# Sanoojan/VFace

Hardware: AMD Instinct MI355X
Metric: swapped frames/sec at 512x512, 50-step DDIM (higher is better)
Workload: dtype f16

## Files before the change

### include/vface_hip.h

```cpp
#ifndef VFACE_HIP_H
#define VFACE_HIP_H

#include <stddef.h>
#include <stdint.h>

#ifdef __cplusplus
extern "C" {
#endif

#define VFACE_ABI_VERSION 8

#define VFACE_OK 0
#define VFACE_ERR_ARG (-1)
#define VFACE_ERR_ALIGN (-2)
#define VFACE_ERR_SHAPE (-3)
#define VFACE_ERR_DTYPE (-4)
#define VFACE_ERR_LAUNCH (-5)
#define VFACE_ERR_WORKSPACE (-6)

#define VFACE_F16 0
#define VFACE_BF16 1

#define VFACE_EPI_GEGLU 1
#define VFACE_EPI_OUT_F32 2
// ... 65 lines not shown

int vface_layernorm(const void* x, int64_t ldx, const float* gamma, const float* beta, void* y, int64_t ldy, int M,
                    int C, float eps, int in_f32, int dtype, void* stream);

int vface_groupnorm_partial_floats(int nimg, int hw, int C, int groups);
int vface_groupnorm_stats(const void* x, int64_t ldx, int nimg, int hw, int C, int groups, float eps, float* partial,
                          float* stats, int in_f32, int dtype, void* stream);
int vface_groupnorm_finalize_cols(const float* colstats, int64_t ld_colstats, int nimg, int hw, int C, int groups, float eps,
                                  float* stats, void* stream);
int vface_groupnorm_coeffs_from_cols(const float* colstats, int64_t ld_colstats, int nimg, int hw, int C, int groups, float eps,
                                     const float* gamma, const float* beta, float* ab, void* stream);
int vface_groupnorm_apply(const void* x, int64_t ldx, const float* stats, const float* gamma, const float* beta,
                          void* y, int64_t ldy, int nimg, int hw, int C, int groups, int silu, int in_f32, int dtype,
                          void* stream);

int vface_flow_warp(const void* src, int64_t ld_src, int64_t fs_src, const void* prev, int64_t ld_prev,
                    const float* flow, const float* flow_prev, void* dst, int64_t ld_dst, int64_t fs_dst, int F,
                    int h, int w, int C, float alpha, float one_minus_alpha, int flags, int32_t* dbg_x0,
                    int32_t* dbg_y0, int dtype, void* stream);

int vface_flow_to_latent(const float* flow_px, float* out, int pairs, int H, int W, int factor, void* stream);

int vface_im2col(const void* X, int64_t ldx, int nimg, int H, int W, int C, int KH, int KW, int stride, int pad_y, int pad_x, void* out,
                 int64_t ldo, int dtype, void* stream);

int64_t vface_channel_stats_partial_floats(int nimg, int hw, int C);
int vface_channel_stats(const void* x, int64_t ldx, int nimg, int hw, int C, float eps, float* partial, float* stats, int dtype,
                        void* stream);

int vface_channel_norm_act(const void* x, int64_t ldx, const float* stats, const void* residual, int64_t ldr, void* y, int64_t ldy,
// ... 125 lines not shown
```

### vface_amd/csrc/capi.cpp

```cpp
#include "../../include/vface_hip.h"

#include <hip/hip_runtime.h>

#include "vface_kernels.hpp"

namespace {
inline hipStream_t S(void* s) { return reinterpret_cast<hipStream_t>(s); }

GemmParams plain_gemm(const void* A, long lda, const void* Wt, long ldw, int M, int N, int K, const float* bias,
                      void* C, long ldc, const void* zeros) {
    GemmParams p{};
    p.mode = 0; p.A = A; p.lda = lda; p.Wt = Wt; p.ldw = ldw; p.Kw = K; p.M = M; p.N = N; p.K = K;
    p.bias = bias; p.C = C; p.ldc = ldc; p.zeros = zeros;
    return p;
}
inline void apply_s32(GemmParams& p, const vface_stream32* s) {
    if (!s) return;
    if (s->residual32) { p.residual = s->residual32; p.ldr = s->ldr32; p.res_f32 = 1; }
    if (s->out32) { p.C32 = s->out32; p.ldc32 = s->ldo32; }
    if (s->in_scale_shift) { p.gn_ab = s->in_scale_shift; p.ld_gn_ab = s->ld_scale_shift; p.gn_silu = s->in_silu ? 1 : 0; }
}
}

extern "C" {
// ... 138 lines not shown
                                  float* stats, void* stream) {
    return vf_launch_gn_finalize_cols(colstats, ld_colstats, nimg, hw, C, groups, eps, stats, S(stream));
}

int vface_groupnorm_coeffs_from_cols(const float* colstats, int64_t ld_colstats, int nimg, int hw, int C, int groups, float eps,
                                     const float* gamma, const float* beta, float* ab, void* stream) {
    return vf_launch_gn_coeffs_cols(colstats, ld_colstats, nimg, hw, C, groups, eps, gamma, beta, ab, S(stream));
}

int vface_groupnorm_apply(const void* x, int64_t ldx, const float* stats, const float* gamma, const float* beta,
                          void* y, int64_t ldy, int nimg, int hw, int C, int groups, int silu, int in_f32, int dtype,
                          void* stream) {
    return vf_launch_gn_apply(x, ldx, stats, gamma, beta, y, ldy, nimg, hw, C, groups, silu, in_f32, dtype, S(stream));
}

int vface_flow_warp(const void* src, int64_t ld_src, int64_t fs_src, const void* prev, int64_t ld_prev,
                    const float* flow, const float* flow_prev, void* dst, int64_t ld_dst, int64_t fs_dst, int F,
                    int h, int w, int C, float alpha, float one_minus_alpha, int flags, int32_t* dbg_x0,
                    int32_t* dbg_y0, int dtype, void* stream) {
    return vf_launch_flow_warp(src, ld_src, fs_src, prev, ld_prev, flow, flow_prev, dst, ld_dst, fs_dst, F, h, w, C,
                               alpha, one_minus_alpha, flags, dbg_x0, dbg_y0, dtype, S(stream));
}

int vface_flow_to_latent(const float* flow_px, float* out, int pairs, int H, int W, int factor, void* stream) {
    return vf_launch_flow_to_latent(flow_px, out, pairs, H, W, factor, S(stream));
}

int vface_im2col(const void* X, int64_t ldx, int nimg, int H, int W, int C, int KH, int KW, int stride, int pad_y, int pad_x, void* out,
                 int64_t ldo, int dtype, void* stream) {
    return vf_launch_im2col(X, ldx, nimg, H, W, C, KH, KW, stride, pad_y, pad_x, out, ldo, dtype, S(stream));
// ... 256 lines not shown
```

### vface_amd/csrc/outconv.hip

```cpp
#include <type_traits>

#include "common.hpp"
#include "vface_kernels.hpp"

namespace {

constexpr int OC_TX = 16, OC_TY = 8;
constexpr int OC_PX = OC_TX + 2, OC_PY = OC_TY + 2;
constexpr int OC_THREADS = 512;
constexpr int OC_ITEMS = OC_PX * OC_PY * 8;
constexpr int OC_NIT = (OC_ITEMS + OC_THREADS - 1) / OC_THREADS;
constexpr int OC_MAXC = 640;
constexpr int OC_PITCH = 64 + 8;

template <class TT, bool IN32, int COUT>
__global__ __launch_bounds__(OC_THREADS) void gn_silu_conv3x3_small_kernel(OutConvParams p) {
    using E = typename TT::elem;
    using V8 = typename TT::v8;
    __shared__ __attribute__((aligned(16))) E patch[OC_PX * OC_PY * OC_PITCH];
    __shared__ float sAB[2 * OC_MAXC];
    static_assert(sizeof(patch) >= 3 * OC_TX * OC_TY * 4 * sizeof(float), "the partial sums are reduced through the patch");
    const int t = threadIdx.x;
    const int tiles_x = (p.W + OC_TX - 1) / OC_TX, tiles_y = (p.H + OC_TY - 1) / OC_TY;
    const int img = blockIdx.x / (tiles_x * tiles_y), tl = blockIdx.x - img * (tiles_x * tiles_y);
    const int ty0 = (tl / tiles_x) * OC_TY, tx0 = (tl % tiles_x) * OC_TX;
    const int pix = t & 127, py = pix >> 4, px = pix & 15;
    const int slice = __builtin_amdgcn_readfirstlane(t >> 7);
    const int oy = ty0 + py, ox = tx0 + px;
    const long img_row0 = (long)img * p.H * p.W;
    float acc[COUT];
#pragma unroll
    for (int o = 0; o < COUT; ++o) acc[o] = 0.f;
    const unsigned* wq = reinterpret_cast<const unsigned*>(p.Wt);
    const int nchunks = p.Cin / 64;
    for (int ch = t; ch < p.Cin; ch += OC_THREADS) {
        const float2 ab = *reinterpret_cast<const float2*>(p.ab + ((long)img * p.ld_ab + ch) * 2);
        sAB[ch] = ab.x; sAB[OC_MAXC + ch] = ab.y;
    }
    using RAW = typename std::conditional<IN32, float4, V8>::type;
    RAW raw[OC_NIT][IN32 ? 2 : 1];
    auto item_row = [&](int i, long& row) -> bool {
        const int it = t + i * OC_THREADS, pp = it >> 3;
        const int iy = ty0 - 1 + pp / OC_PX, ix = tx0 - 1 + pp % OC_PX;
        row = img_row0 + (long)iy * p.W + ix;
        return it < OC_ITEMS && iy >= 0 && iy < p.H && ix >= 0 && ix < p.W;
    };
    auto load_chunk = [&](int c) {
#pragma unroll
// ... 26 lines not shown
                    v[0] = a.x; v[1] = a.y; v[2] = a.z; v[3] = a.w; v[4] = b.x; v[5] = b.y; v[6] = b.z; v[7] = b.w;
                } else {
#pragma unroll
                    for (int j = 0; j < 8; ++j) v[j] = to_f32(raw[i][0][j]);
                }
#pragma unroll
                for (int j = 0; j < 8; ++j) {
                    const float f = v[j] * sAB[c * 64 + g8 * 8 + j] + sAB[OC_MAXC + c * 64 + g8 * 8 + j];
                    o[j] = from_f32<E>(silu_f(f));
                }
            }
            *reinterpret_cast<V8*>(patch + pp * OC_PITCH + g8 * 8) = o;
        }
    };
    load_chunk(0);
    __syncthreads();
    for (int c = 0; c < nchunks; ++c) {
        store_chunk(c);
        __syncthreads();
        if (c + 1 < nchunks) load_chunk(c + 1);
#pragma unroll
        for (int tap = 0; tap < 9; ++tap) {
            const E* pr = patch + ((py + tap / 3) * OC_PX + (px + tap % 3)) * OC_PITCH + slice * 16;
#pragma unroll
            for (int g8 = 0; g8 < 2; ++g8) {
                const V8 xv = *reinterpret_cast<const V8*>(pr + g8 * 8);
#pragma unroll
                for (int o = 0; o < COUT; ++o) {
                    const unsigned* wo = wq + ((long)o * 9 * p.Cin + (long)(c * 9 + tap) * 64 + slice * 16 + g8 * 8) / 2;
#pragma unroll
                    for (int j2 = 0; j2 < 4; ++j2) {
                        const unsigned wpair = wo[j2];
                        if constexpr (std::is_same<TT, F16>::value) {
                            typedef _Float16 h2 __attribute__((ext_vector_type(2)));
                            const h2 xa = {xv[2 * j2], xv[2 * j2 + 1]};
                            acc[o] = __builtin_amdgcn_fdot2(xa, __builtin_bit_cast(h2, wpair), acc[o], false);
                        } else {
                            typedef __bf16 b2 __attribute__((ext_vector_type(2)));
                            const b2 wb = __builtin_bit_cast(b2, wpair);
                            acc[o] = fmaf((float)xv[2 * j2], (float)wb[0], acc[o]);
                            acc[o] = fmaf((float)xv[2 * j2 + 1], (float)wb[1], acc[o]);
                        }
                    }
                }
            }
        }
        __syncthreads();
    }
    float* red = reinterpret_cast<float*>(patch);
    if (slice > 0) {
#pragma unroll
        for (int o = 0; o < COUT; ++o) red[((slice - 1) * 128 + pix) * 4 + o] = acc[o];
    }
    __syncthreads();
    if (slice == 0 && oy < p.H && ox < p.W) {
        float* d = p.out + (img_row0 + (long)oy * p.W + ox) * p.ldo;
#pragma unroll
        for (int o = 0; o < COUT; ++o) {
            const float r = ((acc[o] + red[pix * 4 + o]) + red[(128 + pix) * 4 + o]) + red[(256 + pix) * 4 + o];
            d[o] = r + (p.bias ? p.bias[o] : 0.f);
        }
    }
}

template <class TT>
int launch_t(const OutConvParams& p, hipStream_t stream) {
    const int tiles = ((p.W + OC_TX - 1) / OC_TX) * ((p.H + OC_TY - 1) / OC_TY);
    dim3 grid((unsigned)(p.nimg * tiles));
#define OC_LAUNCH(IN32_, CO_) hipLaunchKernelGGL((gn_silu_conv3x3_small_kernel<TT, IN32_, CO_>), grid, dim3(OC_THREADS), 0, stream, p)
    if (p.Cout == 4) { if (p.in_f32) OC_LAUNCH(true, 4); else OC_LAUNCH(false, 4); }
    else if (p.Cout == 3) { if (p.in_f32) OC_LAUNCH(true, 3); else OC_LAUNCH(false, 3); }
    else return VF_ERR_SHAPE;
#undef OC_LAUNCH
    return hipGetLastError() == hipSuccess ? VF_OK : VF_ERR_LAUNCH;
}

}

bool vf_out_conv_supported(int Cin, int Cout) { return Cin > 0 && Cin <= 640 && (Cin % 64) == 0 && (Cout == 3 || Cout == 4); }

int vf_launch_out_conv(const OutConvParams& p, int dtype, hipStream_t stream) {
    if (!p.x || !p.ab || !p.Wt || !p.out || p.nimg <= 0 || p.H <= 0 || p.W <= 0) return VF_ERR_ARG;
    if (!vf_out_conv_supported(p.Cin, p.Cout)) return VF_ERR_SHAPE;
    if ((p.ldx & (p.in_f32 ? 3 : 7)) || p.ld_ab < p.Cin || p.ldo < p.Cout) return VF_ERR_ALIGN;
    if (((uintptr_t)p.x | (uintptr_t)p.Wt) & 15 || ((uintptr_t)p.ab & 7)) return VF_ERR_ALIGN;
    if (dtype == VF_DTYPE_F16) return launch_t<F16>(p, stream);
    if (dtype == VF_DTYPE_BF16) return launch_t<BF16>(p, stream);
    return VF_ERR_DTYPE;
}
// ... 1 lines not shown
```

### vface_amd/csrc/pointwise.hip

```cpp
#include "common.hpp"
#include "vface_kernels.hpp"

namespace {

template <class TT, bool IN32>
__device__ __forceinline__ void load8(const void* base, long off, float (&f)[8]) {
    if constexpr (IN32) {
        const float4 a = *reinterpret_cast<const float4*>(static_cast<const float*>(base) + off);
        const float4 b = *reinterpret_cast<const float4*>(static_cast<const float*>(base) + off + 4);
        f[0] = a.x; f[1] = a.y; f[2] = a.z; f[3] = a.w; f[4] = b.x; f[5] = b.y; f[6] = b.z; f[7] = b.w;
    } else {
        const typename TT::v8 t = *reinterpret_cast<const typename TT::v8*>(static_cast<const typename TT::elem*>(base) + off);
#pragma unroll
        for (int j = 0; j < 8; ++j) f[j] = to_f32(t[j]);
    }
}

template <class TT, int CH8, bool IN32>
__global__ __launch_bounds__(256) void layernorm_kernel(const void* __restrict__ x, long ldx,
                                                        const float* __restrict__ gamma,
                                                        const float* __restrict__ beta,
                                                        typename TT::elem* __restrict__ y, long ldy, int M, int C,
                                                        float eps) {
    using E = typename TT::elem;
// ... 97 lines not shown
    const int img = blockIdx.x;
    for (int g = threadIdx.x; g < groups; g += blockDim.x) {
        double s = 0.0, q = 0.0;
        for (int c = 0; c < nchunks; ++c) {
            const float* pp = partial + ((long)img * nchunks + c) * 2 * groups;
            s += pp[2 * g]; q += pp[2 * g + 1];
        }
        const double mean = s / count;
        double var = q / count - mean * mean;
        if (var < 0.0) var = 0.0;
        stats[((long)img * groups + g) * 2] = (float)mean;
        stats[((long)img * groups + g) * 2 + 1] = (float)(1.0 / sqrt(var + (double)eps));
    }
}

__global__ __launch_bounds__(64) void gn_finalize_cols_kernel(const float* __restrict__ colstats, long ld, int hw, int C,
                                                              int groups, float eps, float* __restrict__ stats) {
    const int img = blockIdx.y, g = blockIdx.x, lane = threadIdx.x;
    const int cpg = C / groups, spi = hw / 64;
    const int total = cpg * spi;
    double s = 0.0, q = 0.0;
    for (int i = lane; i < total; i += 64) {
        const int sl = i / cpg, c = g * cpg + (i - sl * cpg);
        const float2 v = *reinterpret_cast<const float2*>(colstats + (((long)img * spi + sl) * ld + c) * 2);
        s += v.x; q += v.y;
    }
#pragma unroll
    for (int o = 32; o > 0; o >>= 1) { s += __shfl_xor(s, o, 64); q += __shfl_xor(q, o, 64); }
    if (lane == 0) {
        const double count = (double)hw * cpg;
        const double mean = s / count;
        double var = q / count - mean * mean;
        if (var < 0.0) var = 0.0;
        stats[((long)img * groups + g) * 2] = (float)mean;
        stats[((long)img * groups + g) * 2 + 1] = (float)(1.0 / sqrt(var + (double)eps));
    }
}

__global__ __launch_bounds__(64) void gn_coeffs_cols_kernel(const float* __restrict__ colstats, long ld, int hw, int C, int groups,
                                                            float eps, const float* __restrict__ gamma,
                                                            const float* __restrict__ beta, float* __restrict__ ab) {
    const int img = blockIdx.y, g = blockIdx.x, lane = threadIdx.x;
    const int cpg = C / groups, spi = hw / 64;
    const int total = cpg * spi;
    double s = 0.0, q = 0.0;
    for (int i = lane; i < total; i += 64) {
        const int sl = i / cpg, c = g * cpg + (i - sl * cpg);
        const float2 v = *reinterpret_cast<const float2*>(colstats + (((long)img * spi + sl) * ld + c) * 2);
        s += v.x; q += v.y;
    }
#pragma unroll
    for (int o = 32; o > 0; o >>= 1) { s += __shfl_xor(s, o, 64); q += __shfl_xor(q, o, 64); }
    const double count = (double)hw * cpg;
    const double mean = s / count;
    double var = q / count - mean * mean;
    if (var < 0.0) var = 0.0;
    const float meanf = (float)mean, rstd = (float)(1.0 / sqrt(var + (double)eps));
    for (int c = g * cpg + lane; c < (g + 1) * cpg; c += 64) {
        const float a = rstd * gamma[c];
        *reinterpret_cast<float2*>(ab + ((long)img * C + c) * 2) = make_float2(a, beta[c] - meanf * a);
    }
}

template <class TT, bool IN32, bool DEEP>
__global__ __launch_bounds__(256) void gn_apply_kernel(const void* __restrict__ x, long ldx,
                                                       const float* __restrict__ stats,
                                                       const float* __restrict__ gamma,
                                                       const float* __restrict__ beta,
                                                       typename TT::elem* __restrict__ y, long ldy, int hw, int C,
                                                       int groups, int silu, int pix_per_block) {
    using E = typename TT::elem;
    using V8 = typename TT::v8;
    const int img = blockIdx.y, t = threadIdx.x;
    const int c8 = C / 8, cpg = C / groups;
    const int p0 = blockIdx.x * pix_per_block, p1 = min(hw, p0 + pix_per_block);
// ... 33 lines not shown
            for (int u = 0; u < 4; ++u)
                if (p + u * PP < p1) load8<TT, IN32>(x, xb + (long)(p + u * PP) * ldx + ch * 8, v[u]);
#pragma unroll
            for (int u = 0; u < 4; ++u) {
                if (p + u * PP >= p1) break;
                V8 o;
#pragma unroll
                for (int j = 0; j < 8; ++j) {
                    float f = v[u][j] * a[j] + b[j];
                    if (silu) f = silu_f(f);
                    o[j] = from_f32<E>(f);
                }
                *reinterpret_cast<V8*>(yb + (long)(p + u * PP) * ldy + ch * 8) = o;
            }
        }
    }
}

__device__ __forceinline__ float unnorm_coord(float pos, float d, int size, bool recip) {
    const float v = __fadd_rn(pos, d);
    const float den = (float)max(size - 1, 1);
    const float two_v = __fmul_rn(2.0f, v);
    const float qn = recip ? __fmul_rn(two_v, __fdiv_rn(1.0f, den)) : __fdiv_rn(two_v, den);
    const float g = __fsub_rn(qn, 1.0f);
    float c = __fmul_rn(__fmul_rn(__fadd_rn(g, 1.0f), 0.5f), (float)(size - 1));
    c = fminf((float)(size - 1), fmaxf(c, 0.0f));
    return c;
}

template <class TT>
// ... 765 lines not shown
        using E = typename TT::elem;
        dim3 g((unsigned)nblocks);
        switch (ch8) {
            case 1: hipLaunchKernelGGL((adain_rows_kernel<TT, 1>), g, dim3(256), 0, stream, (const E*)a, lda, (const E*)b, ldb, fused, (long)C, (int)rows, C, partial); break;
            case 2: hipLaunchKernelGGL((adain_rows_kernel<TT, 2>), g, dim3(256), 0, stream, (const E*)a, lda, (const E*)b, ldb, fused, (long)C, (int)rows, C, partial); break;
            case 3: hipLaunchKernelGGL((adain_rows_kernel<TT, 3>), g, dim3(256), 0, stream, (const E*)a, lda, (const E*)b, ldb, fused, (long)C, (int)rows, C, partial); break;
            default: hipLaunchKernelGGL((adain_rows_kernel<TT, 4>), g, dim3(256), 0, stream, (const E*)a, lda, (const E*)b, ldb, fused, (long)C, (int)rows, C, partial); break;
        }
        hipLaunchKernelGGL(adain_reduce_kernel, dim3(1), dim3(256), 0, stream, (const double*)partial, (int)rows, C, inv);
        hipLaunchKernelGGL((adain_scale_kernel<TT>), dim3(grid_for(rows * (C / 8))), dim3(256), 0, stream, (const float*)fused, (long)C,
                           (const float*)inv, (E*)dst, ldd, rows, C);
    });
    return ok();
}

int vf_launch_gn_finalize_cols(const float* colstats, long ld, int nimg, int hw, int C, int groups, float eps, float* stats,
                               hipStream_t stream) {
    if (!colstats || !stats || nimg <= 0 || hw <= 0 || C <= 0 || groups <= 0) return VF_ERR_ARG;
    if ((hw & 63) || (C % groups) || ld < C) return VF_ERR_SHAPE;
    hipLaunchKernelGGL(gn_finalize_cols_kernel, dim3(groups, nimg), dim3(64), 0, stream, colstats, ld, hw, C, groups, eps, stats);
    return ok();
}
```

### vface_amd/csrc/vface_kernels.hpp

```cpp
#pragma once
#include <hip/hip_runtime.h>
#include <stdint.h>

#include <atomic>

struct VfOncePerDevice {
    std::atomic<unsigned long long> done{0};
    bool set_lds(const void* kern, int bytes) {
        int dev = 0;
        if (hipGetDevice(&dev) != hipSuccess) return false;
        const unsigned long long bit = 1ull << (dev & 63);
        if (done.load(std::memory_order_acquire) & bit) return true;
        if (hipFuncSetAttribute(kern, hipFuncAttributeMaxDynamicSharedMemorySize, bytes) != hipSuccess) return false;
        done.fetch_or(bit, std::memory_order_release);
        return true;
    }
};

#include "dispatch.hpp"
bool vf_gemm_variants_built();
int vf_launch_gemm(const GemmParams& p, int dtype, hipStream_t stream);
int vf_launch_conv_patch(const VfGemmPlan& plan, int dtype, hipStream_t stream);
int vf_launch_gemm_big(const VfGemmPlan& plan, int dtype, hipStream_t stream);
int vf_launch_conv_in16(const VfGemmPlan& plan, int dtype, hipStream_t stream);
// ... 68 lines not shown
    const int* v_map;
    void* O; long ldo, bso;
    int B, heads, n, nk, dh;
    float scale;
    int variant;
    unsigned k_bytes, v_bytes;
    int v_sets, set_stride;
    int v_sets_live;
};
int vf_launch_attention(const AttnParams& p, int dtype, hipStream_t stream);

int vf_launch_layernorm(const void* x, long ldx, const float* gamma, const float* beta, void* y, long ldy, int M,
                        int C, float eps, int in_f32, int dtype, hipStream_t stream);
int vf_launch_gn_finalize_cols(const float* colstats, long ld, int nimg, int hw, int C, int groups, float eps, float* stats,
                               hipStream_t stream);
int vf_launch_gn_coeffs_cols(const float* colstats, long ld, int nimg, int hw, int C, int groups, float eps, const float* gamma,
                             const float* beta, float* ab, hipStream_t stream);
int vf_launch_gn_stats(const void* x, long ldx, int nimg, int hw, int C, int groups, float eps, float* partial,
                       float* stats, int in_f32, int dtype, hipStream_t stream);
int vf_gn_partial_floats(int nimg, int hw, int C, int groups);
int vf_launch_gn_apply(const void* x, long ldx, const float* stats, const float* gamma, const float* beta, void* y,
                       long ldy, int nimg, int hw, int C, int groups, int silu, int in_f32, int dtype, hipStream_t stream);
int vf_launch_flow_warp(const void* src, long ld_src, long fs_src, const void* prev, long ld_prev,
                        const float* flow, const float* flow_prev, void* dst, long ld_dst, long fs_dst, int F, int h,
                        int w, int C, float alpha, float one_minus_alpha, int flags, int* dbg_x0, int* dbg_y0, int dtype,
                        hipStream_t stream);
int vf_launch_flow_to_latent(const float* flow_px, float* out, int pairs, int H, int W, int factor, hipStream_t stream);
int vf_launch_im2col(const void* x, long ldx, int nimg, int H, int W, int C, int KH, int KW, int stride, int pad_y, int pad_x, void* out,
                     long ldo, int dtype, hipStream_t stream);
int vf_chan_stats_slices(int hw);
// ... 72 lines not shown
```

### vface_amd/engine.py

```python
from __future__ import annotations

import os

import numpy as np
from dataclasses import dataclass
from typing import Dict, List, Optional, Sequence

import torch

from . import hip, packing
from .replay import _GraphSegments, _StepReplay


@dataclass
class HookCfg:
    switch_on: bool = True
    chunks: int = 3
    fusion: str = "replace"
    flow: Optional[torch.Tensor] = None
    split_ratio_fft: float = 0.8
    alpha: float = 0.8
    flow_gate: str = "reference"


# ... 149 lines not shown
        self.dtype = dtype
        self._device = torch.device(device) if device is not None else None
        self._packed: Dict[str, dict] = {}
        self._maps: Dict[tuple, torch.Tensor] = {}
        self._version = None
        self.halo_exchange = None
        self.halo_flow: Optional[torch.Tensor] = None
        self.halo_hw = None
        self.exchange_events = None
        self.fuse_ffn = os.environ.get("VFACE_FUSE_FFN", "1") != "0"
        self.fuse_front = os.environ.get("VFACE_FUSE_FRONT", "1") != "0"
        self.fuse_tail = os.environ.get("VFACE_FUSE_TAIL", "1") != "0"
        self.fuse_post = os.environ.get("VFACE_FUSE_POST", "1") != "0"
        self.fuse_temb = os.environ.get("VFACE_FUSE_TEMB", "1") != "0"
        self.fuse_out = os.environ.get("VFACE_FUSE_OUT", "1") != "0"
        self.concat32 = os.environ.get("VFACE_CONCAT32", "0") == "1"
        self.interior16 = os.environ.get("VFACE_INTERIOR16", "1") != "0"
        self._shape_ok: Dict[tuple, bool] = {}
        self.live_chunks: Optional[int] = None
        self.share_prefix = False
        self.stream32 = os.environ.get("VFACE_STREAM32", "1") != "0"
        self.fuse_gn = os.environ.get("VFACE_FUSE_GN", "off")
        self._halo_k = 0
        self._a2_lru: Dict[int, tuple] = {}
        self._a2_cache: Optional[tuple] = None
        self._init_replay()
        hip.load()

    @property
    def device(self):
# ... 153 lines not shown
        hip.gemm(a, w["w"], out, M=a.shape[0], N=w["w"].shape[0], K=K, lda=a.stride(0),
                 ldc=out.stride(0) if out is not None else 0, ldw=w["w"].shape[1], bias=w.get("b"), **kw)

    @staticmethod
    def _resid(x) -> dict:
        if isinstance(x, Act):
            if x.t32 is not None:
                return {"residual32": x.t32}
            return {"residual": x.t, "ldr": x.t.stride(0)}
        if x.dtype == torch.float32:
            return {"residual32": x}
        return {"residual": x, "ldr": x.stride(0)}

    def _gn(self, x: Act, gn, eps: float, silu: bool) -> Act:
        src = x.src
        if x.cs is not None:
            st = hip.groupnorm_stats_from_cols(x.cs, nimg=x.N, hw=x.hw, C_=x.C, eps=eps)
        else:
            st = hip.groupnorm_stats(src, nimg=x.N, hw=x.hw, C_=x.C, ldx=src.stride(0), eps=eps)
        y = self._new(x.M, x.C)
        hip.groupnorm_apply(src, st, gn[0], gn[1], y, nimg=x.N, hw=x.hw, C_=x.C, ldx=src.stride(0), ldy=x.C, silu=silu)
        return Act(y, x.N, x.H, x.W)

    def _conv(self, x: Act, w: dict, tgt, stride=1, upsample=False, rowbias=None, residual=None, out_f32=False,
              stream=True, gn_ab=None) -> Act:
        VH, VW = (2 * x.H, 2 * x.W) if upsample else (x.H, x.W)
        OH, OW = (VH - 1) // stride + 1, (VW - 1) // stride + 1
        if tgt is None:
            if out_f32:
                out, cs, o32 = self._new(x.N * OH * OW, w["cout"], torch.float32), None, None
# ... 470 lines not shown
```

### vface_amd/hip.py

```python
from __future__ import annotations

import ctypes as C
import os
from typing import Optional, Tuple

import torch

_HERE = os.path.dirname(os.path.abspath(__file__))
LIB_PATH = os.environ.get("VFACE_HIP_LIB") or os.path.join(_HERE, "lib", "libvface_hip.so")

F16, BF16 = 0, 1
EPI_GEGLU, EPI_OUT_F32 = 1, 2
CONV_PAD_TRAILING = 0x40000
TUNE_NO_PATCH, TUNE_PATCH = 0x80000, 0x100000
TUNE_GN8 = 0x8000000
TUNE_NO_Q8 = 0x4000000
TUNE_PATCH_BN160 = 0x2000000
TUNE_F32_TRANSPOSE = 0x1000000
TUNE_NO_PERSISTENT, TUNE_PERSISTENT = 0x10000, 0x20000
TUNE_BIG_W256, TUNE_BIG_W320 = 0x200000, 0x400000
TUNE_BIG_TILE, TUNE_NO_BIG_TILE = 0x10000000, 0x20000000
FUSION_NONE, FUSION_REPLACE, FUSION_LINEAR = 0, 1, 2

_i64, _i32, _f32, _vp, _sz = C.c_int64, C.c_int, C.c_float, C.c_void_p, C.c_size_t
# ... 17 lines not shown
    "vface_splitk_workspace_bytes": (_i64, [_i32, _i32, _i32, _i32, _i32]),
    "vface_conv_uses_patch_kernel": (C.c_int, [_i32, _i32, _i32, _i32, _i32, _i32, _i32, _i32]),
    "vface_conv3x3_plus_1x1": (C.c_int, [_vp, _i64, _i32, _i32, _i32, _i32, _vp, _i64, _i32, _vp, _i64, _i32, _vp, _vp, _i32,
                                         _vp, _i64, _vp, _i32, _i32, _vp, _i64, _vp, _i64, _vp, _s32p]),
    "vface_upsample2x_conv3x3_phase": (C.c_int, [_vp, _i64, _i32, _i32, _i32, _i32, _vp, _i64, _i32, _i32, _i32, _vp, _vp, _i32,
                                                 _vp, _i64, _vp, _i32, _i32, _vp, _i64, _vp, _s32p]),
    "vface_groupnorm_finalize_cols": (C.c_int, [_vp, _i64, _i32, _i32, _i32, _i32, _f32, _vp, _vp]),
    "vface_attention": (C.c_int, [_vp, _vp, _vp, _i64, _i64, _i64, _i64, _i64, _i64, _vp, _vp, _vp, _i64, _i64, _i32,
                                  _i32, _i32, _i32, _i32, _f32, _i32, _i32, _i32, _vp]),
    "vface_attention_shared_scores_supported": (C.c_int, [_i32, _i32]),
    "vface_layernorm": (C.c_int, [_vp, _i64, _vp, _vp, _vp, _i64, _i32, _i32, _f32, _i32, _i32, _vp]),
    "vface_groupnorm_partial_floats": (C.c_int, [_i32, _i32, _i32, _i32]),
    "vface_groupnorm_stats": (C.c_int, [_vp, _i64, _i32, _i32, _i32, _i32, _f32, _vp, _vp, _i32, _i32, _vp]),
    "vface_groupnorm_coeffs_from_cols": (C.c_int, [_vp, _i64, _i32, _i32, _i32, _i32, _f32, _vp, _vp, _vp, _vp]),
    "vface_groupnorm_apply": (C.c_int, [_vp, _i64, _vp, _vp, _vp, _vp, _i64, _i32, _i32, _i32, _i32, _i32, _i32, _i32, _vp]),
    "vface_flow_warp": (C.c_int, [_vp, _i64, _i64, _vp, _i64, _vp, _vp, _vp, _i64, _i64, _i32, _i32, _i32, _i32, _f32,
                                  _f32, _i32, _vp, _vp, _i32, _vp]),
    "vface_flow_to_latent": (C.c_int, [_vp, _vp, _i32, _i32, _i32, _i32, _vp]),
    "vface_im2col": (C.c_int, [_vp, _i64, _i32, _i32, _i32, _i32, _i32, _i32, _i32, _i32, _i32, _vp, _i64, _i32, _vp]),
    "vface_channel_stats_partial_floats": (_i64, [_i32, _i32, _i32]),
    "vface_channel_stats": (C.c_int, [_vp, _i64, _i32, _i32, _i32, _f32, _vp, _vp, _i32, _vp]),
    "vface_channel_norm_act": (C.c_int, [_vp, _i64, _vp, _vp, _i64, _vp, _i64, _vp, _i64, _i64, _i32, _i32, _i32, _i32, _vp]),
    "vface_gru_gate": (C.c_int, [_vp, _i64, _vp, _vp, _i64, _vp, _i64, _i64, _i32, _i32, _vp]),
    "vface_gru_update": (C.c_int, [_vp, _i64, _vp, _i64, _vp, _vp, _i64, _vp, _i64, _i64, _i32, _i32, _vp]),
    "vface_avgpool2_f32": (C.c_int, [_vp, _vp, _i64, _i32, _i32, _vp]),
    "vface_corr_lookup": (C.c_int, [_vp, _vp, _vp, _i32, _vp, _i32, _i32, _f32, _vp, _i64, _i64, _i32, _vp]),
    "vface_flow_update": (C.c_int, [_vp, _vp, _i64, _vp, _i64, _vp, _i64, _vp, _i64, _i64, _i32, _vp]),
    "vface_convex_upsample": (C.c_int, [_vp, _i64, _vp, _vp, _i32, _i32, _i32, _f32, _vp]),
    "vface_frame_to_u8": (C.c_int, [_vp, _vp, _i32, _i32, _i32, _i32, _vp]),
    "vface_resample_u8": (C.c_int, [_vp, _vp, _i32, _i32, _i32, _i32, _i32, _vp, _vp, _i32, _vp]),
# ... 228 lines not shown
                               groups: int = 32, eps: float = 1e-5) -> torch.Tensor:
    ab = torch.empty(nimg, C_, 2, dtype=torch.float32, device=colstats.device)
    rc = load().vface_groupnorm_coeffs_from_cols(_p(colstats), colstats.stride(0) // 2, nimg, hw, C_, groups, eps, _p(gamma),
                                                 _p(beta), _p(ab), _stream())
    _check(rc, "vface_groupnorm_coeffs_from_cols")
    return ab


def groupnorm_apply(x: torch.Tensor, stats: torch.Tensor, gamma: torch.Tensor, beta: torch.Tensor, out: torch.Tensor,
                    *, nimg: int, hw: int, C_: int, ldx: int, ldy: int, groups: int = 32, silu: bool = False):
    rc = load().vface_groupnorm_apply(_p(x), ldx, _p(stats), _p(gamma), _p(beta), _p(out), ldy, nimg, hw, C_, groups,
                                      int(silu), int(x.dtype == torch.float32), dtype_code(out.dtype), _stream())
    _check(rc, "vface_groupnorm_apply")


def flow_warp(src: torch.Tensor, dst: torch.Tensor, flow: Optional[torch.Tensor], *, F: int, h: int, w: int, C_: int,
              ld_src: int, fs_src: int, ld_dst: int, fs_dst: int, alpha: float, prev=None, ld_prev: int = 0,
              flow_prev=None, cuda_recip_div: bool = False, dbg_x0=None, dbg_y0=None):
    rc = load().vface_flow_warp(_p(src), ld_src, fs_src, _p(prev), ld_prev, _p(flow), _p(flow_prev), _p(dst), ld_dst,
                                fs_dst, F, h, w, C_, float(alpha), float(1.0 - alpha), int(cuda_recip_div),
                                _p(dbg_x0), _p(dbg_y0), dtype_code(src.dtype), _stream())
    _check(rc, "vface_flow_warp")


def flow_to_latent(flow_px: torch.Tensor, factor: int = 8) -> torch.Tensor:
    if flow_px.dim() != 4 or flow_px.shape[1] != 2:
        raise VFaceHipError(f"flow must be [pairs, 2, H, W]; got {tuple(flow_px.shape)}")
    f = flow_px.to(dtype=torch.float32).contiguous()
    P, _, H, W = f.shape
    out = torch.empty(P, 2, H // factor, W // factor, dtype=torch.float32, device=f.device)
# ... 500 lines not shown
```

### vface_amd/replay.py

```python
from __future__ import annotations

import os
import warnings
from typing import Dict, Optional

import torch

from . import hip


def _timed(cur, fn):
    e0, e1 = torch.cuda.Event(enable_timing=True), torch.cuda.Event(enable_timing=True)
    e0.record(cur)
    out = fn()
    e1.record(cur)
    e1.synchronize()
    return e0.elapsed_time(e1), out


class _GraphSegments:

    def __init__(self, engine, inner):
        self.engine, self.inner = engine, inner
        self.stream = torch.cuda.Stream()
# ... 123 lines not shown
        self.split_streams = int(os.environ.get("VFACE_STREAMS", "2"))
        self._split_state: "Dict[tuple, dict]" = {}
        self._split_pair = None
        self._split_verified = False
        self.split_overlap = None
        self.split_selfcheck = os.environ.get("VFACE_SPLIT_SELFCHECK", "1") != "0"
        self.split_checked: Dict[str, bool] = {}
        self.split_timing: Dict[tuple, tuple] = {}
        self._split_off: set = set()

    def _hooked_cfgs(self):
        for kind, _, mod in self.unet.layer_table():
            if kind == "st":
                yield getattr(mod.transformer_blocks[0].attn1, "_vface_cfg", None)

    _GRAPH_SWITCHES = ("stream32", "fuse_gn", "fuse_ffn", "fuse_front", "fuse_tail", "fuse_post", "fuse_temb", "fuse_out", "concat32",
                       "interior16", "live_chunks", "share_prefix")

    def _hook_signature(self):
        sig, flows = [], []
        for cfg in self._hooked_cfgs():
            if cfg is None:
                sig.append(None)
                continue
            fl = cfg.flow
            if fl is not None and not any(f is fl for f in flows):
                flows.append(fl)
            sig.append((cfg.switch_on, cfg.chunks, cfg.fusion, cfg.split_ratio_fft, cfg.alpha, cfg.flow_gate,
                        (next(i for i, f in enumerate(flows) if f is fl), tuple(fl.shape)) if fl is not None else None))
        return tuple(sig), flows

    _SPLIT_SAFE = ("replace", "fft", "fft_vfixed", "mix")
# ... 325 lines not shown
```

Baseline: 8.284.

## Fuse small-map groupnorm stats with apply and move output conv to MFMA

Adds a kernel that turns column statistics into group mean/rstd inside the apply kernel for small feature maps (hw<=256, fp32 input), so the separate finalize launch and its stats buffer are no longer needed. It is enabled by default through an engine switch that also feeds the graph signature. Separately, the GN+SiLU 3x3 output conv is rewritten to stage its weights in dynamic LDS and use MFMA instead of per-thread dot products, which drops the cross-slice reduction. The cost is redundant per-block stats recomputation and larger LDS use, which may lower occupancy.

```diff
diff --git a/include/vface_hip.h b/include/vface_hip.h
--- a/include/vface_hip.h
+++ b/include/vface_hip.h
@@ -103,6 +103,10 @@
                           void* y, int64_t ldy, int nimg, int hw, int C, int groups, int silu, int in_f32, int dtype,
                           void* stream);
 
+int vface_groupnorm_cols_apply(const float* colstats, int64_t ld_colstats, const void* x, int64_t ldx, const float* gamma,
+                               const float* beta, void* y, int64_t ldy, float* stats, int nimg, int hw, int C, int groups,
+                               float eps, int silu, int in_f32, int dtype, void* stream);
+
 int vface_flow_warp(const void* src, int64_t ld_src, int64_t fs_src, const void* prev, int64_t ld_prev,
                     const float* flow, const float* flow_prev, void* dst, int64_t ld_dst, int64_t fs_dst, int F,
                     int h, int w, int C, float alpha, float one_minus_alpha, int flags, int32_t* dbg_x0,
diff --git a/vface_amd/csrc/capi.cpp b/vface_amd/csrc/capi.cpp
--- a/vface_amd/csrc/capi.cpp
+++ b/vface_amd/csrc/capi.cpp
@@ -176,6 +176,13 @@
     return vf_launch_gn_apply(x, ldx, stats, gamma, beta, y, ldy, nimg, hw, C, groups, silu, in_f32, dtype, S(stream));
 }
 
+int vface_groupnorm_cols_apply(const float* colstats, int64_t ld_colstats, const void* x, int64_t ldx, const float* gamma,
+                               const float* beta, void* y, int64_t ldy, float* stats, int nimg, int hw, int C, int groups,
+                               float eps, int silu, int in_f32, int dtype, void* stream) {
+    return vf_launch_gn_cols_apply(colstats, ld_colstats, x, ldx, gamma, beta, y, ldy, stats, nimg, hw, C, groups, eps, silu, in_f32,
+                                   dtype, S(stream));
+}
+
 int vface_flow_warp(const void* src, int64_t ld_src, int64_t fs_src, const void* prev, int64_t ld_prev,
                     const float* flow, const float* flow_prev, void* dst, int64_t ld_dst, int64_t fs_dst, int F,
                     int h, int w, int C, float alpha, float one_minus_alpha, int flags, int32_t* dbg_x0,
diff --git a/vface_amd/csrc/outconv.hip b/vface_amd/csrc/outconv.hip
--- a/vface_amd/csrc/outconv.hip
+++ b/vface_amd/csrc/outconv.hip
@@ -19,19 +19,13 @@
     using V8 = typename TT::v8;
     __shared__ __attribute__((aligned(16))) E patch[OC_PX * OC_PY * OC_PITCH];
     __shared__ float sAB[2 * OC_MAXC];
-    static_assert(sizeof(patch) >= 3 * OC_TX * OC_TY * 4 * sizeof(float), "the partial sums are reduced through the patch");
+    extern __shared__ __attribute__((aligned(16))) unsigned char oc_dyn[];
+    E* wl = reinterpret_cast<E*>(oc_dyn);
     const int t = threadIdx.x;
     const int tiles_x = (p.W + OC_TX - 1) / OC_TX, tiles_y = (p.H + OC_TY - 1) / OC_TY;
     const int img = blockIdx.x / (tiles_x * tiles_y), tl = blockIdx.x - img * (tiles_x * tiles_y);
     const int ty0 = (tl / tiles_x) * OC_TY, tx0 = (tl % tiles_x) * OC_TX;
-    const int pix = t & 127, py = pix >> 4, px = pix & 15;
-    const int slice = __builtin_amdgcn_readfirstlane(t >> 7);
-    const int oy = ty0 + py, ox = tx0 + px;
     const long img_row0 = (long)img * p.H * p.W;
-    float acc[COUT];
-#pragma unroll
-    for (int o = 0; o < COUT; ++o) acc[o] = 0.f;
-    const unsigned* wq = reinterpret_cast<const unsigned*>(p.Wt);
     const int nchunks = p.Cin / 64;
     for (int ch = t; ch < p.Cin; ch += OC_THREADS) {
         const float2 ab = *reinterpret_cast<const float2*>(p.ab + ((long)img * p.ld_ab + ch) * 2);
@@ -88,65 +82,66 @@
         }
     };
     load_chunk(0);
+    for (int i = t; i < COUT * 9 * p.Cin / 8; i += OC_THREADS)
+        reinterpret_cast<V8*>(wl)[i] = reinterpret_cast<const V8*>(p.Wt)[i];
+    if (t < 4) {
+        V8 z;
+#pragma unroll
+        for (int j = 0; j < 8; ++j) z[j] = (E)0.0f;
+        reinterpret_cast<V8*>(wl + COUT * 9 * p.Cin)[t] = z;
+    }
     __syncthreads();
+    const int lane = t & 63, row = __builtin_amdgcn_readfirstlane(t >> 6);
+    const int fm = lane & 15, fk = (lane >> 4) * 8;
+    f4_t acc = {0.f, 0.f, 0.f, 0.f};
+    const int wstep = fm < COUT ? 1 : 0;
+    const E* wrow = wl + (fm < COUT ? fm : COUT) * 9 * p.Cin + fk;
     for (int c = 0; c < nchunks; ++c) {
         store_chunk(c);
         __syncthreads();
         if (c + 1 < nchunks) load_chunk(c + 1);
 #pragma unroll
         for (int tap = 0; tap < 9; ++tap) {
-            const E* pr = patch + ((py + tap / 3) * OC_PX + (px + tap % 3)) * OC_PITCH + slice * 16;
+            const E* pr = patch + ((row + tap / 3) * OC_PX + (fm + tap % 3)) * OC_PITCH + fk;
+            const E* wr = wrow + wstep * ((c * 9 + tap) * 64);
 #pragma unroll
-            for (int g8 = 0; g8 < 2; ++g8) {
-                const V8 xv = *reinterpret_cast<const V8*>(pr + g8 * 8);
-#pragma unroll
-                for (int o = 0; o < COUT; ++o) {
-                    const unsigned* wo = wq + ((long)o * 9 * p.Cin + (long)(c * 9 + tap) * 64 + slice * 16 + g8 * 8) / 2;
-#pragma unroll
-                    for (int j2 = 0; j2 < 4; ++j2) {
-                        const unsigned wpair = wo[j2];
-                        if constexpr (std::is_same<TT, F16>::value) {
-                            typedef _Float16 h2 __attribute__((ext_vector_type(2)));
-                            const h2 xa = {xv[2 * j2], xv[2 * j2 + 1]};
-                            acc[o] = __builtin_amdgcn_fdot2(xa, __builtin_bit_cast(h2, wpair), acc[o], false);
-                        } else {
-                            typedef __bf16 b2 __attribute__((ext_vector_type(2)));
-                            const b2 wb = __builtin_bit_cast(b2, wpair);
-                            acc[o] = fmaf((float)xv[2 * j2], (float)wb[0], acc[o]);
-                            acc[o] = fmaf((float)xv[2 * j2 + 1], (float)wb[1], acc[o]);
-                        }
-                    }
-                }
+            for (int h = 0; h < 2; ++h) {
+                const V8 av = *reinterpret_cast<const V8*>(pr + h * 32);
+                const V8 bv = *reinterpret_cast<const V8*>(wr + wstep * (h * 32));
+                acc = TT::mfma32(av, bv, acc);
             }
         }
         __syncthreads();
     }
-    float* red = reinterpret_cast<float*>(patch);
-    if (slice > 0) {
+    const int oy = ty0 + row;
+    if (fm < COUT && oy < p.H) {
+        const float bn = p.bias ? p.bias[fm] : 0.f;
 #pragma unroll
-        for (int o = 0; o < COUT; ++o) red[((slice - 1) * 128 + pix) * 4 + o] = acc[o];
-    }
-    __syncthreads();
-    if (slice == 0 && oy < p.H && ox < p.W) {
-        float* d = p.out + (img_row0 + (long)oy * p.W + ox) * p.ldo;
-#pragma unroll
-        for (int o = 0; o < COUT; ++o) {
-            const float r = ((acc[o] + red[pix * 4 + o]) + red[(128 + pix) * 4 + o]) + red[(256 + pix) * 4 + o];
-            d[o] = r + (p.bias ? p.bias[o] : 0.f);
+        for (int i = 0; i < 4; ++i) {
+            const int ox = tx0 + (lane >> 4) * 4 + i;
+            if (ox < p.W) p.out[(img_row0 + (long)oy * p.W + ox) * p.ldo + fm] = acc[i] + bn;
         }
     }
+}
+
+template <class TT, bool IN32, int COUT>
+int launch_one(const OutConvParams& p, dim3 grid, hipStream_t stream) {
+    auto kern = gn_silu_conv3x3_small_kernel<TT, IN32, COUT>;
+    const size_t wbytes = ((size_t)COUT * 9 * p.Cin + 32) * sizeof(typename TT::elem);
+    static VfOncePerDevice attr_set;
+    if (wbytes > 32 * 1024 && !attr_set.set_lds(reinterpret_cast<const void*>(kern), (COUT * 9 * OC_MAXC + 32) * (int)sizeof(typename TT::elem)))
+        return VF_ERR_LAUNCH;
+    hipLaunchKernelGGL(kern, grid, dim3(OC_THREADS), wbytes, stream, p);
+    return hipGetLastError() == hipSuccess ? VF_OK : VF_ERR_LAUNCH;
 }
 
 template <class TT>
 int launch_t(const OutConvParams& p, hipStream_t stream) {
     const int tiles = ((p.W + OC_TX - 1) / OC_TX) * ((p.H + OC_TY - 1) / OC_TY);
     dim3 grid((unsigned)(p.nimg * tiles));
-#define OC_LAUNCH(IN32_, CO_) hipLaunchKernelGGL((gn_silu_conv3x3_small_kernel<TT, IN32_, CO_>), grid, dim3(OC_THREADS), 0, stream, p)
-    if (p.Cout == 4) { if (p.in_f32) OC_LAUNCH(true, 4); else OC_LAUNCH(false, 4); }
-    else if (p.Cout == 3) { if (p.in_f32) OC_LAUNCH(true, 3); else OC_LAUNCH(false, 3); }
-    else return VF_ERR_SHAPE;
-#undef OC_LAUNCH
-    return hipGetLastError() == hipSuccess ? VF_OK : VF_ERR_LAUNCH;
+    if (p.Cout == 4) return p.in_f32 ? launch_one<TT, true, 4>(p, grid, stream) : launch_one<TT, false, 4>(p, grid, stream);
+    if (p.Cout == 3) return p.in_f32 ? launch_one<TT, true, 3>(p, grid, stream) : launch_one<TT, false, 3>(p, grid, stream);
+    return VF_ERR_SHAPE;
 }
 
 }
diff --git a/vface_amd/csrc/pointwise.hip b/vface_amd/csrc/pointwise.hip
--- a/vface_amd/csrc/pointwise.hip
+++ b/vface_amd/csrc/pointwise.hip
@@ -135,26 +135,45 @@
     }
 }
 
+template <int NG>
+__device__ __forceinline__ void gn_group_stats_cols(const float* __restrict__ colstats, long ld, int img, int g, int gstep, int cpg,
+                                                    int spi, int hw, float eps, int lane, float (&meanf)[NG], float (&rstdf)[NG]) {
+    const int total = cpg * spi;
+    double s[NG], q[NG];
+#pragma unroll
+    for (int k = 0; k < NG; ++k) s[k] = q[k] = 0.0;
+    for (int i = lane; i < total; i += 64) {
+        const int sl = i / cpg, cc = i - sl * cpg;
+#pragma unroll
+        for (int k = 0; k < NG; ++k) {
+            const float2 v = *reinterpret_cast<const float2*>(colstats + (((long)img * spi + sl) * ld + (g + k * gstep) * cpg + cc) * 2);
+            s[k] += v.x; q[k] += v.y;
+        }
+    }
+#pragma unroll
+    for (int o = 32; o > 0; o >>= 1) {
+#pragma unroll
+        for (int k = 0; k < NG; ++k) { s[k] += __shfl_xor(s[k], o, 64); q[k] += __shfl_xor(q[k], o, 64); }
+    }
+    const double count = (double)hw * cpg;
+#pragma unroll
+    for (int k = 0; k < NG; ++k) {
+        const double mean = s[k] / count;
+        double var = q[k] / count - mean * mean;
+        if (var < 0.0) var = 0.0;
+        meanf[k] = (float)mean;
+        rstdf[k] = (float)(1.0 / sqrt(var + (double)eps));
+    }
+}
+
 __global__ __launch_bounds__(64) void gn_finalize_cols_kernel(const float* __restrict__ colstats, long ld, int hw, int C,
                                                               int groups, float eps, float* __restrict__ stats) {
     const int img = blockIdx.y, g = blockIdx.x, lane = threadIdx.x;
-    const int cpg = C / groups, spi = hw / 64;
-    const int total = cpg * spi;
-    double s = 0.0, q = 0.0;
-    for (int i = lane; i < total; i += 64) {
-        const int sl = i / cpg, c = g * cpg + (i - sl * cpg);
-        const float2 v = *reinterpret_cast<const float2*>(colstats + (((long)img * spi + sl) * ld + c) * 2);
-        s += v.x; q += v.y;
-    }
-#pragma unroll
-    for (int o = 32; o > 0; o >>= 1) { s += __shfl_xor(s, o, 64); q += __shfl_xor(q, o, 64); }
+    float mean[1], rstd[1];
+    gn_group_stats_cols<1>(colstats, ld, img, g, 0, C / groups, hw / 64, hw, eps, lane, mean, rstd);
     if (lane == 0) {
-        const double count = (double)hw * cpg;
-        const double mean = s / count;
-        double var = q / count - mean * mean;
-        if (var < 0.0) var = 0.0;
-        stats[((long)img * groups + g) * 2] = (float)mean;
-        stats[((long)img * groups + g) * 2 + 1] = (float)(1.0 / sqrt(var + (double)eps));
+        stats[((long)img * groups + g) * 2] = mean[0];
+        stats[((long)img * groups + g) * 2 + 1] = rstd[0];
     }
 }
 
@@ -162,24 +181,12 @@
                                                             float eps, const float* __restrict__ gamma,
                                                             const float* __restrict__ beta, float* __restrict__ ab) {
     const int img = blockIdx.y, g = blockIdx.x, lane = threadIdx.x;
-    const int cpg = C / groups, spi = hw / 64;
-    const int total = cpg * spi;
-    double s = 0.0, q = 0.0;
-    for (int i = lane; i < total; i += 64) {
-        const int sl = i / cpg, c = g * cpg + (i - sl * cpg);
-        const float2 v = *reinterpret_cast<const float2*>(colstats + (((long)img * spi + sl) * ld + c) * 2);
-        s += v.x; q += v.y;
-    }
-#pragma unroll
-    for (int o = 32; o > 0; o >>= 1) { s += __shfl_xor(s, o, 64); q += __shfl_xor(q, o, 64); }
-    const double count = (double)hw * cpg;
-    const double mean = s / count;
-    double var = q / count - mean * mean;
-    if (var < 0.0) var = 0.0;
-    const float meanf = (float)mean, rstd = (float)(1.0 / sqrt(var + (double)eps));
+    const int cpg = C / groups;
+    float meanf[1], rstd[1];
+    gn_group_stats_cols<1>(colstats, ld, img, g, 0, cpg, hw / 64, hw, eps, lane, meanf, rstd);
     for (int c = g * cpg + lane; c < (g + 1) * cpg; c += 64) {
-        const float a = rstd * gamma[c];
-        *reinterpret_cast<float2*>(ab + ((long)img * C + c) * 2) = make_float2(a, beta[c] - meanf * a);
+        const float a = rstd[0] * gamma[c];
+        *reinterpret_cast<float2*>(ab + ((long)img * C + c) * 2) = make_float2(a, beta[c] - meanf[0] * a);
     }
 }
 
@@ -243,6 +250,88 @@
                 *reinterpret_cast<V8*>(yb + (long)(p + u * PP) * ldy + ch * 8) = o;
             }
         }
+    }
+}
+
+#ifndef VF_GNF_BLOCKS
+#define VF_GNF_BLOCKS 1024
+#endif
+template <class TT, bool IN32>
+__device__ __forceinline__ void gn_load_trip(const void* __restrict__ x, long xoff, long ldx, int p, int PP, int p1, float (&v)[4][8]) {
+#pragma unroll
+    for (int u = 0; u < 4; ++u)
+        if (p + u * PP < p1) load8<TT, IN32>(x, xoff + (long)(p + u * PP) * ldx, v[u]);
+}
+
+template <class TT, bool IN32>
+__global__ __launch_bounds__(256) void gn_cols_apply_kernel(const float* __restrict__ colstats, long ld, const void* __restrict__ x,
+                                                            long ldx, const float* __restrict__ gamma,
+                                                            const float* __restrict__ beta, typename TT::elem* __restrict__ y,
+                                                            long ldy, float* __restrict__ stats, int hw, int C, int groups, int gpw,
+                                                            float eps, int silu, int pix_per_block) {
+    using E = typename TT::elem;
+    using V8 = typename TT::v8;
+    __shared__ float st[2 * 64];
+    const int img = blockIdx.y, t = threadIdx.x;
+    const int ncb = groups / gpw, pblk = blockIdx.x / ncb, g0 = (blockIdx.x - pblk * ncb) * gpw;
+    const int cpg = C / groups;
+    const int CPB = gpw * cpg / 8, PP = 256 / CPB;
+    const int lanep = t / CPB, c0 = g0 * cpg + (t - lanep * CPB) * 8;
+    const int p0 = pblk * pix_per_block, p1 = min(hw, p0 + pix_per_block);
+    const bool live = lanep < PP;
+    const long xoff = (long)img * hw * ldx + c0;
+    E* yb = y + (long)img * hw * ldy + c0;
+    int p = p0 + lanep;
+    float v[4][8], gm[8], bt[8];
+    if (live) {
+        gn_load_trip<TT, IN32>(x, xoff, ldx, p, PP, p1, v);
+#pragma unroll
+        for (int j = 0; j < 8; ++j) { gm[j] = gamma[c0 + j]; bt[j] = beta[c0 + j]; }
+    }
+    auto keep = [&](int gi, float mean, float rstd) {
+        st[2 * gi] = mean; st[2 * gi + 1] = rstd;
+        if (stats && pblk == 0) {
+            stats[((long)img * groups + g0 + gi) * 2] = mean;
+            stats[((long)img * groups + g0 + gi) * 2 + 1] = rstd;
+        }
+    };
+    const int wave = t >> 6, lane = t & 63;
+    if (gpw == 8) {
+        float mean[2], rstd[2];
+        gn_group_stats_cols<2>(colstats, ld, img, g0 + wave, 4, cpg, hw / 64, hw, eps, lane, mean, rstd);
+        if (lane == 0) { keep(wave, mean[0], rstd[0]); keep(wave + 4, mean[1], rstd[1]); }
+    } else {
+        for (int gi = wave; gi < gpw; gi += 4) {
+            float mean[1], rstd[1];
+            gn_group_stats_cols<1>(colstats, ld, img, g0 + gi, 0, cpg, hw / 64, hw, eps, lane, mean, rstd);
+            if (lane == 0) keep(gi, mean[0], rstd[0]);
+        }
+    }
+    __syncthreads();
+    if (!live) return;
+    float a[8], b[8];
+#pragma unroll
+    for (int j = 0; j < 8; ++j) {
+        const int g = (c0 + j) / cpg - g0;
+        a[j] = st[2 * g + 1] * gm[j];
+        b[j] = bt[j] - st[2 * g] * a[j];
+    }
+    for (;;) {
+#pragma unroll
+        for (int u = 0; u < 4; ++u) {
+            if (p + u * PP >= p1) break;
+            V8 o;
+#pragma unroll
+            for (int j = 0; j < 8; ++j) {
+                float f = v[u][j] * a[j] + b[j];
+                if (silu) f = silu_f(f);
+                o[j] = from_f32<E>(f);
+            }
+            *reinterpret_cast<V8*>(yb + (long)(p + u * PP) * ldy) = o;
+        }
+        p += 4 * PP;
+        if (p >= p1) break;
+        gn_load_trip<TT, IN32>(x, xoff, ldx, p, PP, p1, v);
     }
 }
 
@@ -1038,6 +1127,25 @@
     return ok();
 }
 
+int vf_launch_gn_cols_apply(const float* colstats, long ld, const void* x, long ldx, const float* gamma, const float* beta, void* y,
+                            long ldy, float* stats, int nimg, int hw, int C, int groups, float eps, int silu, int in_f32, int dtype,
+                            hipStream_t stream) {
+    if (!colstats || !x || !gamma || !beta || !y || nimg <= 0 || hw <= 0 || C <= 0 || groups <= 0) return VF_ERR_ARG;
+    if ((hw & 63) || hw > 256 || (C & 7) || groups > 64 || C % groups || ld < C) return VF_ERR_SHAPE;
+    if ((ldx & (in_f32 ? 3 : 7)) || (ldy & 7) || (((uintptr_t)x | (uintptr_t)y) & 15)) return VF_ERR_ALIGN;
+    const int gpw = (groups & 7) ? groups : 8;
+    if (gpw * (C / groups) > 2048) return VF_ERR_SHAPE;
+    int ppb = hw;
+    while (ppb > 32 && (long)nimg * (groups / gpw) * ((hw + ppb - 1) / ppb) < VF_GNF_BLOCKS) ppb >>= 1;
+    dim3 grid((groups / gpw) * ((hw + ppb - 1) / ppb), nimg);
+    DISPATCH_DTYPE(dtype, {
+        using E = typename TT::elem;
+        if (in_f32) hipLaunchKernelGGL((gn_cols_apply_kernel<TT, true>), grid, dim3(256), 0, stream, colstats, ld, x, ldx, gamma, beta, (E*)y, ldy, stats, hw, C, groups, gpw, eps, silu, ppb);
+        else hipLaunchKernelGGL((gn_cols_apply_kernel<TT, false>), grid, dim3(256), 0, stream, colstats, ld, x, ldx, gamma, beta, (E*)y, ldy, stats, hw, C, groups, gpw, eps, silu, ppb);
+    });
+    return ok();
+}
+
 int vf_launch_gn_finalize_cols(const float* colstats, long ld, int nimg, int hw, int C, int groups, float eps, float* stats,
                                hipStream_t stream) {
     if (!colstats || !stats || nimg <= 0 || hw <= 0 || C <= 0 || groups <= 0) return VF_ERR_ARG;
diff --git a/vface_amd/csrc/vface_kernels.hpp b/vface_amd/csrc/vface_kernels.hpp
--- a/vface_amd/csrc/vface_kernels.hpp
+++ b/vface_amd/csrc/vface_kernels.hpp
@@ -106,6 +106,9 @@
                         int C, float eps, int in_f32, int dtype, hipStream_t stream);
 int vf_launch_gn_finalize_cols(const float* colstats, long ld, int nimg, int hw, int C, int groups, float eps, float* stats,
                                hipStream_t stream);
+int vf_launch_gn_cols_apply(const float* colstats, long ld, const void* x, long ldx, const float* gamma, const float* beta, void* y,
+                            long ldy, float* stats, int nimg, int hw, int C, int groups, float eps, int silu, int in_f32, int dtype,
+                            hipStream_t stream);
 int vf_launch_gn_coeffs_cols(const float* colstats, long ld, int nimg, int hw, int C, int groups, float eps, const float* gamma,
                              const float* beta, float* ab, hipStream_t stream);
 int vf_launch_gn_stats(const void* x, long ldx, int nimg, int hw, int C, int groups, float eps, float* partial,
diff --git a/vface_amd/engine.py b/vface_amd/engine.py
--- a/vface_amd/engine.py
+++ b/vface_amd/engine.py
@@ -187,6 +187,7 @@
         self.fuse_post = os.environ.get("VFACE_FUSE_POST", "1") != "0"
         self.fuse_temb = os.environ.get("VFACE_FUSE_TEMB", "1") != "0"
         self.fuse_out = os.environ.get("VFACE_FUSE_OUT", "1") != "0"
+        self.gn_fused_small = os.environ.get("VFACE_GN_FUSED_SMALL", "1") != "0"
         self.concat32 = os.environ.get("VFACE_CONCAT32", "0") == "1"
         self.interior16 = os.environ.get("VFACE_INTERIOR16", "1") != "0"
         self._shape_ok: Dict[tuple, bool] = {}
@@ -370,6 +371,11 @@
 
     def _gn(self, x: Act, gn, eps: float, silu: bool) -> Act:
         src = x.src
+        if self.gn_fused_small and x.cs is not None and x.hw <= 256 and src.dtype == torch.float32 and x.C % 256 == 0:
+            y = self._new(x.M, x.C)
+            hip.groupnorm_cols_apply(x.cs, src, gn[0], gn[1], y, nimg=x.N, hw=x.hw, C_=x.C, ldx=src.stride(0), ldy=x.C, eps=eps,
+                                     silu=silu)
+            return Act(y, x.N, x.H, x.W)
         if x.cs is not None:
             st = hip.groupnorm_stats_from_cols(x.cs, nimg=x.N, hw=x.hw, C_=x.C, eps=eps)
         else:
diff --git a/vface_amd/hip.py b/vface_amd/hip.py
--- a/vface_amd/hip.py
+++ b/vface_amd/hip.py
@@ -55,6 +55,8 @@
     "vface_groupnorm_stats": (C.c_int, [_vp, _i64, _i32, _i32, _i32, _i32, _f32, _vp, _vp, _i32, _i32, _vp]),
     "vface_groupnorm_coeffs_from_cols": (C.c_int, [_vp, _i64, _i32, _i32, _i32, _i32, _f32, _vp, _vp, _vp, _vp]),
     "vface_groupnorm_apply": (C.c_int, [_vp, _i64, _vp, _vp, _vp, _vp, _i64, _i32, _i32, _i32, _i32, _i32, _i32, _i32, _vp]),
+    "vface_groupnorm_cols_apply": (C.c_int, [_vp, _i64, _vp, _i64, _vp, _vp, _vp, _i64, _vp, _i32, _i32, _i32, _i32, _f32, _i32, _i32, _i32,
+                                             _vp]),
     "vface_flow_warp": (C.c_int, [_vp, _i64, _i64, _vp, _i64, _vp, _vp, _vp, _i64, _i64, _i32, _i32, _i32, _i32, _f32,
                                   _f32, _i32, _vp, _vp, _i32, _vp]),
     "vface_flow_to_latent": (C.c_int, [_vp, _vp, _i32, _i32, _i32, _i32, _vp]),
@@ -313,6 +315,15 @@
     _check(rc, "vface_groupnorm_apply")
 
 
+def groupnorm_cols_apply(colstats: torch.Tensor, x: torch.Tensor, gamma: torch.Tensor, beta: torch.Tensor, out: torch.Tensor, *,
+                         nimg: int, hw: int, C_: int, ldx: int, ldy: int, groups: int = 32, eps: float = 1e-5, silu: bool = False,
+                         stats: Optional[torch.Tensor] = None):
+    rc = load().vface_groupnorm_cols_apply(_p(colstats), colstats.stride(0) // 2, _p(x), ldx, _p(gamma), _p(beta), _p(out), ldy,
+                                           _p(stats), nimg, hw, C_, groups, eps, int(silu), int(x.dtype == torch.float32),
+                                           dtype_code(out.dtype), _stream())
+    _check(rc, "vface_groupnorm_cols_apply")
+
+
 def flow_warp(src: torch.Tensor, dst: torch.Tensor, flow: Optional[torch.Tensor], *, F: int, h: int, w: int, C_: int,
               ld_src: int, fs_src: int, ld_dst: int, fs_dst: int, alpha: float, prev=None, ld_prev: int = 0,
               flow_prev=None, cuda_recip_div: bool = False, dbg_x0=None, dbg_y0=None):
diff --git a/vface_amd/replay.py b/vface_amd/replay.py
--- a/vface_amd/replay.py
+++ b/vface_amd/replay.py
@@ -161,8 +161,8 @@
             if kind == "st":
                 yield getattr(mod.transformer_blocks[0].attn1, "_vface_cfg", None)
 
-    _GRAPH_SWITCHES = ("stream32", "fuse_gn", "fuse_ffn", "fuse_front", "fuse_tail", "fuse_post", "fuse_temb", "fuse_out", "concat32",
-                       "interior16", "live_chunks", "share_prefix")
+    _GRAPH_SWITCHES = ("stream32", "fuse_gn", "fuse_ffn", "fuse_front", "fuse_tail", "fuse_post", "fuse_temb", "fuse_out", "gn_fused_small",
+                       "concat32", "interior16", "live_chunks", "share_prefix")
 
     def _hook_signature(self):
         sig, flows = [], []
```

After: 8.325, median of 5. About the same (+0.5%).
